# LFY1998/IPDM-PyTorch

Measured on AMD Instinct MI355X. Metric: CT slices/s (full proj+img partial-diffusion sample), higher is better.
Workload: dtype f32

## Files before the change

### ipdm-pytorch_amd/csrc/attn.hip

```cpp
#include <cstdlib>
#include "unet_kernels.h"

using namespace ipdm;

typedef float f32x16 __attribute__((ext_vector_type(16)));
typedef float f32x4 __attribute__((ext_vector_type(4)));
typedef float f32x2 __attribute__((ext_vector_type(2)));

namespace {

constexpr int KV = 64;
constexpr int KP = 68;
constexpr int VP = 68;
constexpr float LOG2E = 1.4426950408889634f;

__device__ inline int crow(int r, int h) { return (r & 3) + 8 * (r >> 2) + 4 * h; }

__device__ inline float halves_max(float x)
{
    float a = x, b = x;
    asm volatile("s_nop 1\n\tv_permlane32_swap_b32 %0, %1" : "+v"(a), "+v"(b));
    return fmaxf(a, b);
}
__device__ inline float halves_sum(float x)
{
    float a = x, b = x;
    asm volatile("s_nop 1\n\tv_permlane32_swap_b32 %0, %1" : "+v"(a), "+v"(b));
    return a + b;
}

template <int D, int QT>
__global__ void __launch_bounds__(256, 2) attention_kernel(const float *__restrict__ qkv, float *__restrict__ out,
                                                           int heads, int T, float scale)
{
    __shared__ __attribute__((aligned(16))) float k_lds[KV * KP];
    __shared__ __attribute__((aligned(16))) float v_lds[D * VP];
    const int tid = threadIdx.x, lane = tid & 63, wave = tid >> 6;
    const int l31 = lane & 31, lh = lane >> 5;
    const int bh = blockIdx.y;
    const int b = bh / heads, head = bh % heads;
    const float *qp = qkv + ((size_t)b * heads * 3 * D + (size_t)head * 3 * D) * T;
    const float *kp = qp + (size_t)D * T;
    const float *vp = qp + (size_t)2 * D * T;
    const int t0 = blockIdx.x * (128 * QT) + wave * (32 * QT);
    constexpr int HP = D / 2;

    float qreg[QT][HP];
#pragma unroll
    for (int qt = 0; qt < QT; ++qt) {
        const int t = t0 + qt * 32 + l31;
#pragma unroll
        for (int p = 0; p < HP; ++p) qreg[qt][p] = t < T ? qp[(size_t)(lh * HP + p) * T + t] * scale : 0.0f;
    }

    constexpr int CB = D / 32;
    f32x16 o[QT][CB];
#pragma unroll
    for (int qt = 0; qt < QT; ++qt)
#pragma unroll
        for (int cb = 0; cb < CB; ++cb)
#pragma unroll
            for (int r = 0; r < 16; ++r) o[qt][cb][r] = 0.0f;
    float m_run[QT], l_run[QT];
#pragma unroll
    for (int qt = 0; qt < QT; ++qt) { m_run[qt] = -INFINITY; l_run[qt] = 0.0f; }

    for (int s0 = 0; s0 < T; s0 += KV) {
        __syncthreads();
#pragma unroll
        for (int e = 0; e < (D * KV) / 256; ++e) {
            const int idx = tid + e * 256;
            const int c = idx / KV, s = idx % KV;
            const bool ok = (s0 + s) < T;
            k_lds[s * KP + c] = ok ? kp[(size_t)c * T + s0 + s] * scale : 0.0f;
            v_lds[c * VP + s] = ok ? vp[(size_t)c * T + s0 + s] : 0.0f;
        }
        __syncthreads();
#pragma unroll
        for (int sb = 0; sb < KV / 32; ++sb) {
            if (s0 + sb * 32 >= T) break;
            f32x16 sacc[QT];
#pragma unroll
            for (int qt = 0; qt < QT; ++qt)
#pragma unroll
                for (int r = 0; r < 16; ++r) sacc[qt][r] = 0.0f;
            const float *krow = k_lds + (sb * 32 + l31) * KP + lh * HP;
#pragma unroll
            for (int g = 0; g < HP / 4; ++g) {
                const f32x4 kv = *reinterpret_cast<const f32x4 *>(krow + g * 4);
#pragma unroll
                for (int j = 0; j < 4; ++j)
#pragma unroll
                    for (int qt = 0; qt < QT; ++qt)
                        sacc[qt] = __builtin_amdgcn_mfma_f32_32x32x2f32(kv[j], qreg[qt][g * 4 + j], sacc[qt], 0, 0, 0);
            }
            const bool ragged = s0 + sb * 32 + 32 > T;
#pragma unroll
            for (int qt = 0; qt < QT; ++qt) {
                if (ragged) {
#pragma unroll
                    for (int r = 0; r < 16; ++r)
                        if (s0 + sb * 32 + crow(r, lh) >= T) sacc[qt][r] = -INFINITY;
                }
                float mx = sacc[qt][0];
#pragma unroll
                for (int r = 1; r < 16; ++r) mx = fmaxf(mx, sacc[qt][r]);
                mx = halves_max(mx);
                const float m_new = fmaxf(m_run[qt], mx);
                const float mb = -m_new * LOG2E;
                const float alpha = __builtin_amdgcn_exp2f((m_run[qt] - m_new) * LOG2E);
                float rs = 0.0f;
#pragma unroll
                for (int r = 0; r < 16; ++r) {
                    sacc[qt][r] = __builtin_amdgcn_exp2f(fmaf(sacc[qt][r], LOG2E, mb));
                    rs += sacc[qt][r];
                }
                rs = halves_sum(rs);
                l_run[qt] = l_run[qt] * alpha + rs;
                m_run[qt] = m_new;
                if (__any(alpha != 1.0f)) {
#pragma unroll
                    for (int cb = 0; cb < CB; ++cb)
#pragma unroll
                        for (int r = 0; r < 16; ++r) o[qt][cb][r] *= alpha;
                }
            }
#pragma unroll
            for (int cb = 0; cb < CB; ++cb) {
                const float *vrow = v_lds + (cb * 32 + l31) * VP + sb * 32 + 4 * lh;
#pragma unroll
                for (int g = 0; g < 4; ++g) {
                    const f32x4 vv = *reinterpret_cast<const f32x4 *>(vrow + 8 * g);
#pragma unroll
                    for (int j = 0; j < 4; ++j)
#pragma unroll
                        for (int qt = 0; qt < QT; ++qt)
                            o[qt][cb] = __builtin_amdgcn_mfma_f32_32x32x2f32(vv[j], sacc[qt][4 * g + j], o[qt][cb], 0, 0, 0);
                }
            }
        }
    }
    float *op = out + ((size_t)b * heads * D + (size_t)head * D) * T;
#pragma unroll
    for (int qt = 0; qt < QT; ++qt) {
        const int t = t0 + qt * 32 + l31;
        if (t < T) {
            const float inv = 1.0f / l_run[qt];
#pragma unroll
            for (int cb = 0; cb < CB; ++cb)
#pragma unroll
                for (int r = 0; r < 16; ++r) {
                    const int c = cb * 32 + crow(r, lh);
                    op[(size_t)c * T + t] = o[qt][cb][r] * inv;
                }
        }
    }
}

struct SliceWeights { float a, b; };
__device__ inline SliceWeights slice_weights(float &M, float m_k)
{
    const float Mn = fmaxf(M, m_k);
    SliceWeights w;
    w.a = __builtin_amdgcn_exp2f((M - Mn) * LOG2E);
    w.b = __builtin_amdgcn_exp2f((m_k - Mn) * LOG2E);
    M = Mn;
    return w;
}
__device__ inline float slice_fold(float acc, float v, SliceWeights w) { return fmaf(acc, w.a, v * w.b); }

template <int D, int QT, bool ZSEQ = false>
__global__ void __launch_bounds__(512, ZSEQ ? 2 : 1) attention_ws_kernel(const float *__restrict__ qkv, float *__restrict__ out,
                                                           int heads, int T, float scale, int zsplit, float *__restrict__ part, int zseq)
{
    extern __shared__ __attribute__((aligned(16))) float smem[];
    constexpr int STAGE = KV * KP + D * VP;
    const int bh = blockIdx.y;
    const int b = bh / heads, head = bh % heads;
    const float *qp = qkv + ((size_t)b * heads * 3 * D + (size_t)head * 3 * D) * T;
    const int ntiles = (T + KV - 1) / KV;
    const int nslice = ZSEQ ? zseq : zsplit;
    const int tps = (ntiles + nslice - 1) / nslice;
    const int it0 = ZSEQ ? 0 : blockIdx.z * tps, it1 = ZSEQ ? ntiles : min(ntiles, it0 + tps);

    if (threadIdx.x >= 256) {
        const int tid = threadIdx.x - 256;
        constexpr int NE = (D * KV) / 256;
        const int s_l = tid % KV, c_l = tid / KV;
        const __amdgpu_buffer_rsrc_t rs = __builtin_amdgcn_make_buffer_rsrc((void *)qp, 0, 3 * D * T * 4, 0x00020000);
        int voff[NE];
#pragma unroll
        for (int e = 0; e < NE; ++e) voff[e] = ((c_l + (256 / KV) * e) * T + s_l) * 4;
        const int k_base = s_l * KP + c_l, v_base = c_l * VP + s_l;
        for (int it = it0; it < it1; ++it) {
            const int s0 = it * KV;
            float *k_lds = smem + (it & 1) * STAGE, *v_lds = k_lds + KV * KP;
            const bool last = s0 + KV > T;
            float kr[NE], vr[NE];
            if (!last) {
#pragma unroll
                for (int e = 0; e < NE; ++e) {
                    kr[e] = __builtin_bit_cast(float, __builtin_amdgcn_raw_buffer_load_b32(rs, voff[e], (D * T + s0) * 4, 0));
                    vr[e] = __builtin_bit_cast(float, __builtin_amdgcn_raw_buffer_load_b32(rs, voff[e], (2 * D * T + s0) * 4, 0));
                }
            } else {
#pragma unroll
                for (int e = 0; e < NE; ++e) {
                    const int vo = s0 + s_l >= T ? 0x7fffffff : voff[e];
                    kr[e] = __builtin_bit_cast(float, __builtin_amdgcn_raw_buffer_load_b32(rs, vo, (D * T + s0) * 4, 0));
                    vr[e] = __builtin_bit_cast(float, __builtin_amdgcn_raw_buffer_load_b32(rs, vo, (2 * D * T + s0) * 4, 0));
                }
            }
#pragma unroll
            for (int e = 0; e < NE; ++e) {
                k_lds[k_base + (256 / KV) * e] = kr[e];
                v_lds[v_base + (256 / KV) * e * VP] = vr[e];
            }
            __syncthreads();
        }
        return;
    }

    const int tid = threadIdx.x, lane = tid & 63, wave = tid >> 6;
    const int l31 = lane & 31, lh = lane >> 5;
    const int t0 = blockIdx.x * (128 * QT) + wave * (32 * QT);
    constexpr int HP = D / 2;
    float qreg[QT][HP];
#pragma unroll
    for (int qt = 0; qt < QT; ++qt) {
        const int t = t0 + qt * 32 + l31;
#pragma unroll
        for (int p = 0; p < HP; ++p) qreg[qt][p] = t < T ? qp[(size_t)(lh * HP + p) * T + t] * (scale * scale) : 0.0f;
    }
    constexpr int CB = D / 32;
    f32x16 o[QT][CB];
#pragma unroll
    for (int qt = 0; qt < QT; ++qt)
#pragma unroll
        for (int cb = 0; cb < CB; ++cb)
#pragma unroll
            for (int r = 0; r < 16; ++r) o[qt][cb][r] = 0.0f;
    float m_run[QT], l_run[QT];
#pragma unroll
    for (int qt = 0; qt < QT; ++qt) { m_run[qt] = -INFINITY; l_run[qt] = 0.0f; }
    static_assert(!ZSEQ || QT == 1, "attention: key slices exist for 32-query waves");
    f32x16 num[ZSEQ ? CB : 1];
    float M_all = -INFINITY, den = 0.0f;
#pragma unroll
    for (int cb = 0; cb < (ZSEQ ? CB : 1); ++cb)
#pragma unroll
        for (int r = 0; r < 16; ++r) num[cb][r] = 0.0f;
    int slice_end = it0 + tps;

    for (int it = it0; it < it1; ++it) {
        const int s0 = it * KV;
        __syncthreads();
        const float *k_lds = smem + (it & 1) * STAGE, *v_lds = k_lds + KV * KP;
#pragma unroll
        for (int sb = 0; sb < KV / 32; ++sb) {
            if (s0 + sb * 32 >= T) break;
            f32x16 sacc[QT];
#pragma unroll
            for (int qt = 0; qt < QT; ++qt)
#pragma unroll
                for (int r = 0; r < 16; ++r) sacc[qt][r] = 0.0f;
            const float *krow = k_lds + (sb * 32 + l31) * KP + lh * HP;
#pragma unroll
            for (int g = 0; g < HP / 4; ++g) {
                const f32x4 kv = *reinterpret_cast<const f32x4 *>(krow + g * 4);
#pragma unroll
                for (int j = 0; j < 4; ++j)
#pragma unroll
                    for (int qt = 0; qt < QT; ++qt)
                        sacc[qt] = __builtin_amdgcn_mfma_f32_32x32x2f32(kv[j], qreg[qt][g * 4 + j], sacc[qt], 0, 0, 0);
            }
            const bool ragged = s0 + sb * 32 + 32 > T;
#pragma unroll
            for (int qt = 0; qt < QT; ++qt) {
                if (ragged) {
#pragma unroll
                    for (int r = 0; r < 16; ++r)
                        if (s0 + sb * 32 + crow(r, lh) >= T) sacc[qt][r] = -INFINITY;
                }
                float mx = sacc[qt][0];
#pragma unroll
                for (int r = 1; r < 16; ++r) mx = fmaxf(mx, sacc[qt][r]);
                mx = halves_max(mx);
                const float m_new = fmaxf(m_run[qt], mx);
                const float mb = -m_new * LOG2E;
                const float alpha = __builtin_amdgcn_exp2f((m_run[qt] - m_new) * LOG2E);
                f32x2 rs2 = {0.0f, 0.0f};
#pragma unroll
                for (int r = 0; r < 16; r += 2) {
                    f32x2 v = f32x2{sacc[qt][r], sacc[qt][r + 1]} * LOG2E + mb;
                    v[0] = __builtin_amdgcn_exp2f(v[0]);
                    v[1] = __builtin_amdgcn_exp2f(v[1]);
                    sacc[qt][r] = v[0];
                    sacc[qt][r + 1] = v[1];
                    rs2 += v;
                }
                float rs = halves_sum(rs2[0] + rs2[1]);
                l_run[qt] = l_run[qt] * alpha + rs;
                m_run[qt] = m_new;
                if (__any(alpha != 1.0f)) {
#pragma unroll
                    for (int cb = 0; cb < CB; ++cb)
#pragma unroll
                        for (int r = 0; r < 16; ++r) o[qt][cb][r] *= alpha;
                }
            }
#pragma unroll
            for (int cb = 0; cb < CB; ++cb) {
                const float *vrow = v_lds + (cb * 32 + l31) * VP + sb * 32 + 4 * lh;
#pragma unroll
                for (int g = 0; g < 4; ++g) {
                    const f32x4 vv = *reinterpret_cast<const f32x4 *>(vrow + 8 * g);
#pragma unroll
                    for (int j = 0; j < 4; ++j)
#pragma unroll
                        for (int qt = 0; qt < QT; ++qt)
                            o[qt][cb] = __builtin_amdgcn_mfma_f32_32x32x2f32(vv[j], sacc[qt][4 * g + j], o[qt][cb], 0, 0, 0);
                }
            }
        }
        if constexpr (ZSEQ) if (it + 1 == slice_end || it + 1 == it1) {
            const SliceWeights w = slice_weights(M_all, m_run[0]);
            den = slice_fold(den, l_run[0], w);
#pragma unroll
            for (int cb = 0; cb < CB; ++cb)
#pragma unroll
                for (int r = 0; r < 16; ++r) { num[cb][r] = slice_fold(num[cb][r], o[0][cb][r], w); o[0][cb][r] = 0.0f; }
            m_run[0] = -INFINITY;
            l_run[0] = 0.0f;
            slice_end += tps;
        }
    }
    if (zsplit > 1) {
        float *pp = part + ((size_t)blockIdx.z * gridDim.y + bh) * (D + 2) * T;
#pragma unroll
        for (int qt = 0; qt < QT; ++qt) {
            const int t = t0 + qt * 32 + l31;
            if (t < T) {
#pragma unroll
                for (int cb = 0; cb < CB; ++cb)
#pragma unroll
                    for (int r = 0; r < 16; ++r) pp[(size_t)(cb * 32 + crow(r, lh)) * T + t] = o[qt][cb][r];
                if (lh == 0) { pp[(size_t)D * T + t] = m_run[qt]; pp[(size_t)(D + 1) * T + t] = l_run[qt]; }
            }
        }
        return;
    }
    float *op = out + ((size_t)b * heads * D + (size_t)head * D) * T;
#pragma unroll
    for (int qt = 0; qt < QT; ++qt) {
        const int t = t0 + qt * 32 + l31;
        if (t < T) {
            constexpr bool seq = ZSEQ;
            const float inv = 1.0f / (seq ? den : l_run[qt]);
#pragma unroll
            for (int cb = 0; cb < CB; ++cb)
#pragma unroll
                for (int r = 0; r < 16; ++r) {
                    const int c = cb * 32 + crow(r, lh);
                    op[(size_t)c * T + t] = (seq ? num[seq ? cb : 0][r] : o[qt][cb][r]) * inv;
                }
        }
    }
}

template <int D>
__global__ void __launch_bounds__(256) attention_combine_kernel(const float *__restrict__ part, float *__restrict__ out, int T, int Z, int ntiles)
{
    const int t = blockIdx.x * 256 + threadIdx.x, bh = blockIdx.y, c0 = blockIdx.z * 16;
    if (t >= T) return;
    const size_t slice = (size_t)gridDim.y * (D + 2) * T;
    const float *p = part + (size_t)bh * (D + 2) * T;
    const int tps = (ntiles + Z - 1) / Z;
    SliceWeights w[8];
    float M = -INFINITY, den = 0.0f;
#pragma unroll
    for (int z = 0; z < 8; ++z)
        if (z < Z && z * tps < ntiles) {
            w[z] = slice_weights(M, p[z * slice + (size_t)D * T + t]);
            den = slice_fold(den, p[z * slice + (size_t)(D + 1) * T + t], w[z]);
        }
    const float inv = 1.0f / den;
#pragma unroll 4
    for (int c = c0; c < c0 + 16; ++c) {
        float acc = 0.0f;
#pragma unroll
        for (int z = 0; z < 8; ++z)
            if (z < Z && z * tps < ntiles) acc = slice_fold(acc, p[z * slice + (size_t)c * T + t], w[z]);
        out[((size_t)bh * D + c) * T + t] = acc * inv;
    }
}

int attention_kv_split(int B, int heads, int d, int T)
{
    const bool off = opt(OPT_ATTN_NO_KVSPLIT) != 0;
    (void)B;
    if (off || d != 64) return 1;
    const long wg = (long)cdiv(T, 128) * heads;
    if (wg > 128) return 1;
    const int ntiles = cdiv(T, KV);
    int Z = wg <= 32 ? 8 : (wg <= 64 ? 4 : 2);
    if (Z > ntiles / 2) Z = ntiles / 2;
    return Z < 2 ? 1 : Z;
}

}

namespace ipdm {

size_t attention_scratch_floats(int B, int heads, int d, int T)
{
    const int Z = attention_kv_split(B, heads, d, T);
    return Z > 1 ? (size_t)Z * B * heads * (d + 2) * T : 0;
}

int attention_launch(const float *qkv, float *out, int B, int heads, int d, int T, hipStream_t st, float *scratch)
{
    IPDM_REQUIRE(qkv && out && B > 0 && heads > 0 && T > 0, "attention: bad argument");
    if (d != 64 && d != 32) { set_error("attention: head dim %d unsupported (kernel is specialised for 64 and 32)", d); return IPDM_ERR_UNSUPPORTED; }
    const float scale = (float)(1.0 / sqrt(sqrt((double)d)));
    const bool prof = prof_enabled();
    if (prof) prof_before(2, st);
    const bool legacy = opt(OPT_ATTN_LEGACY) != 0;
    if (d == 64 && !legacy) {
        constexpr size_t lds = (size_t)2 * (KV * KP + 64 * VP) * sizeof(float);
        if (int rc = ensure_dynamic_lds((const void *)attention_ws_kernel<64, 1>, lds)) return rc;
        if (int rc = ensure_dynamic_lds((const void *)attention_ws_kernel<64, 2>, lds)) return rc;
        if (int rc = ensure_dynamic_lds((const void *)attention_ws_kernel<64, 1, true>, lds)) return rc;
        const long wg2 = (long)cdiv(T, 256) * B * heads, wg1 = (long)cdiv(T, 128) * B * heads;
        const auto eff = [](long wg) { return (double)wg / (double)(((wg + 255) / 256) * 256); };
        const int Z = scratch ? attention_kv_split(B, heads, d, T) : 1;
        const bool q2 = Z == 1 && wg2 >= 256 && eff(wg2) >= eff(wg1) - 0.03;
        const bool no_seq = opt(OPT_ATTN_NO_ZSEQ) != 0;
        const bool seq = Z >= 4 && !no_seq && wg1 >= 192;
        dim3 grid(cdiv(T, q2 ? 256 : 128), B * heads, seq ? 1 : Z);
        if (q2) hipLaunchKernelGGL((attention_ws_kernel<64, 2>), grid, dim3(512), lds, st, qkv, out, heads, T, scale, 1, (float *)nullptr, 1);
        else if (seq) hipLaunchKernelGGL((attention_ws_kernel<64, 1, true>), grid, dim3(512), lds, st, qkv, out, heads, T, scale, 1, (float *)nullptr, Z);
        else hipLaunchKernelGGL((attention_ws_kernel<64, 1>), grid, dim3(512), lds, st, qkv, out, heads, T, scale, Z, scratch, 1);
        if (Z > 1 && !seq)
            hipLaunchKernelGGL((attention_combine_kernel<64>), dim3(cdiv(T, 256), B * heads, 4), dim3(256), 0, st, scratch, out, T, Z, cdiv(T, KV));
    } else if (d == 64) {
        const long wg2 = (long)cdiv(T, 256) * B * heads;
        const bool q2 = wg2 >= 512 && (wg2 % 512 == 0 || wg2 >= 4 * 512);
        dim3 grid(cdiv(T, q2 ? 256 : 128), B * heads);
        if (q2) hipLaunchKernelGGL((attention_kernel<64, 2>), grid, dim3(256), 0, st, qkv, out, heads, T, scale);
        else hipLaunchKernelGGL((attention_kernel<64, 1>), grid, dim3(256), 0, st, qkv, out, heads, T, scale);
    } else {
        dim3 grid(cdiv(T, 128), B * heads);
        hipLaunchKernelGGL((attention_kernel<32, 1>), grid, dim3(256), 0, st, qkv, out, heads, T, scale);
    }
    if (prof) prof_after(2, 4.0 * B * heads * (double)T * T * d, st);
    IPDM_LAUNCH_CHECK();
    return IPDM_OK;
}

}

extern "C" int32_t ipdm_attention_kernel_code(int32_t d)
{
    return (d == 64 && !ipdm::opt(ipdm::OPT_ATTN_LEGACY)) ? 1 : 0;
}

extern "C" int ipdm_op_attention(const float *d_qkv, float *d_out, int32_t B, int32_t heads, int32_t d, int32_t T,
                                 void *stream)
{
    float *scratch = nullptr;
    if (ipdm::attention_scratch_floats(B, heads, d, T)) {
        IPDM_HIP_CHECK(hipMalloc((void **)&scratch, ipdm::attention_scratch_floats(B, heads, d, T) * sizeof(float)));
    }
    const int rc = ipdm::attention_launch(d_qkv, d_out, B, heads, d, T, (hipStream_t)stream, scratch);
    if (scratch) {
        (void)hipStreamSynchronize((hipStream_t)stream);
        (void)hipFree(scratch);
    }
    return rc;
}
```

### ipdm-pytorch_amd/csrc/common.h

```cpp
#pragma once
#include <hip/hip_runtime.h>
#include <cstdarg>
#include <cstdio>
#include <cstring>
#include <string>
#include <vector>
#include "../../include/ipdm_hip.h"

namespace ipdm {

void set_error(const char *fmt, ...);

#define IPDM_HIP_CHECK(expr)                                                                   \
    do {                                                                                       \
        hipError_t e_ = (expr);                                                                \
        if (e_ != hipSuccess) {                                                                \
            ipdm::set_error("%s failed: %s (%s:%d)", #expr, hipGetErrorString(e_), __FILE__,  \
                            __LINE__);                                                         \
            return IPDM_ERR_HIP;                                                               \
        }                                                                                      \
    } while (0)

#define IPDM_REQUIRE(cond, ...)                   \
    do {                                          \
        if (!(cond)) {                            \
            ipdm::set_error(__VA_ARGS__);         \
            return IPDM_ERR_INVALID;              \
        }                                         \
    } while (0)

#define IPDM_LAUNCH_CHECK() IPDM_HIP_CHECK(hipGetLastError())

static inline int cdiv(long a, long b) { return (int)((a + b - 1) / b); }
static inline size_t align_up(size_t v, size_t a) { return (v + a - 1) / a * a; }

enum Opt {
    OPT_CONV_NO_UP2,
    OPT_CONV_NO_WUP2,
    OPT_CONV_LEGACY, OPT_CONV1X1_LEGACY, OPT_CONVS2_LEGACY,
    OPT_CONV_NO_DIRECT, OPT_DIRECT_NO_PLANAR, OPT_DIRECT_MAX_CIN, OPT_DIRECT_NO_S2, OPT_DIRECT_NO_SKIP_FUSE,
    OPT_CONV_DBG, OPT_CONV_VEC4_STRICT, OPT_CONV_NO_SPLITK, OPT_CONV_NO_WINO, OPT_WINO_V1, OPT_WINO2_MIN_TILES, OPT_CONV1X1_NO_QUARTER, OPT_CONV_NO_PW, OPT_PW_ITEM, OPT_PW_FORCE,
    OPT_CONV_NM,
    OPT_GN_TWO_STAGE, OPT_GN_UNFUSED,
    OPT_UNET_TRANSPOSE,
    OPT_ATTN_NO_KVSPLIT, OPT_ATTN_LEGACY, OPT_ATTN_NO_ZSEQ,
    OPT_ART_PER_VIEW,
    OPT_CONV_BF16X3,
    OPT_COUNT
};
int opt(Opt o);
bool opt_per_call(int o);
const char *opt_name(int o);
void opt_snapshot(int (&dst)[OPT_COUNT]);
int opt_changed_since(const int (&rec)[OPT_COUNT]);
std::vector<int> opt_per_call_values();

int ensure_dynamic_lds(const void *kernel, size_t bytes);
int device_cu_count();

__device__ inline double wave_sum(double v)
{
#pragma unroll
    for (int o = 32; o > 0; o >>= 1) v += __shfl_down(v, o, 64);
    return v;
}
__device__ inline float wave_sum(float v)
{
#pragma unroll
    for (int o = 32; o > 0; o >>= 1) v += __shfl_down(v, o, 64);
    return v;
}
__device__ inline float wave_max(float v)
{
#pragma unroll
    for (int o = 32; o > 0; o >>= 1) v = fmaxf(v, __shfl_down(v, o, 64));
    return v;
}

}
```

### ipdm-pytorch_amd/csrc/common.hip

```cpp
#include <cctype>
#include <cstdlib>
#include <mutex>
#include <strings.h>
#include <set>
#include <utility>
#include "common.h"

namespace ipdm {
static thread_local char g_err[512] = "";
void set_error(const char *fmt, ...)
{
    va_list ap;
    va_start(ap, fmt);
    vsnprintf(g_err, sizeof(g_err), fmt, ap);
    va_end(ap);
}

namespace {
std::mutex g_attr_mu;
std::set<std::pair<const void *, int>> g_attr_done;
int g_cus[64];
}

namespace {
struct OptDef { const char *name; int def; bool per_call; int lo = 0, hi = 1; };
const OptDef g_opt_def[OPT_COUNT] = {
    {"conv_no_up2", 0, true},
    {"conv_no_wup2", 0, true},
    {"conv_legacy", 0, false}, {"conv1x1_legacy", 0, false}, {"convs2_legacy", 0, false},
    {"conv_no_direct", 0, false}, {"direct_no_planar", 0, false},
    {"direct_max_cin", 160, false, 0, 160},
    {"direct_no_s2", 0, false}, {"direct_no_skip_fuse", 0, true},
    {"conv_dbg", 0, true, 0, 0x3ff}, {"conv_vec4_strict", 0, false}, {"conv_no_splitk", 0, false},
    {"conv_no_wino", 0, true}, {"wino_v1", 0, true}, {"wino2_min_tiles", 192, true, 0, 1 << 24},
    {"conv1x1_no_quarter", 0, true}, {"conv_no_pw", 0, true}, {"pw_item", 0, true, 0, 2}, {"pw_force", 0, true}, {"conv_nm", 0, true, 0, 2},
    {"gn_two_stage", 0, true}, {"gn_unfused", 0, true},
    {"unet_transpose", -1, true, -1, 1},
    {"attn_no_kvsplit", 0, false}, {"attn_legacy", 0, false}, {"attn_no_zseq", 0, true},
    {"art_per_view", 0, true},
    {"conv_bf16x3", 0, true},
};
bool opt_value_ok(int i, int v)
{
    return v >= g_opt_def[i].lo && v <= g_opt_def[i].hi;
}
std::mutex g_opt_mu;
int g_opt_val[OPT_COUNT];
bool g_opt_init = false;

void opt_init_locked()
{
    if (g_opt_init) return;
    for (int i = 0; i < OPT_COUNT; ++i) {
        char env[64] = "IPDM_";
        size_t n = 5;
        for (const char *c = g_opt_def[i].name; *c && n + 1 < sizeof(env); ++c) env[n++] = (char)toupper((unsigned char)*c);
        env[n] = 0;
        const char *e = getenv(env);
        g_opt_val[i] = g_opt_def[i].def;
        if (e) {
            char *end = nullptr;
            const long v = strtol(e, &end, 10);
            const int want = (end != e) ? (int)v : 1;
            if (opt_value_ok(i, want)) g_opt_val[i] = want;
            else fprintf(stderr, "libipdm_hip: %s=%s is outside the option's range [%d, %d]: ignored\n", env, e, g_opt_def[i].lo, g_opt_def[i].hi);
        }
    }
    g_opt_init = true;
}
}

int opt(Opt o)
{
    std::lock_guard<std::mutex> lk(g_opt_mu);
    opt_init_locked();
    return g_opt_val[o];
}
bool opt_per_call(int o) { return g_opt_def[o].per_call; }
const char *opt_name(int o) { return g_opt_def[o].name; }
void opt_snapshot(int (&dst)[OPT_COUNT])
{
    std::lock_guard<std::mutex> lk(g_opt_mu);
    opt_init_locked();
    for (int i = 0; i < OPT_COUNT; ++i) dst[i] = g_opt_val[i];
}
std::vector<int> opt_per_call_values()
{
    std::lock_guard<std::mutex> lk(g_opt_mu);
    opt_init_locked();
    std::vector<int> v;
    for (int i = 0; i < OPT_COUNT; ++i)
        if (g_opt_def[i].per_call) v.push_back(g_opt_val[i]);
    return v;
}
int opt_changed_since(const int (&rec)[OPT_COUNT])
{
    std::lock_guard<std::mutex> lk(g_opt_mu);
    opt_init_locked();
    for (int i = 0; i < OPT_COUNT; ++i)
        if (!g_opt_def[i].per_call && g_opt_val[i] != rec[i]) return i;
    return -1;
}
static int opt_find(const char *name)
{
    if (!name) return -1;
    if (!strncmp(name, "IPDM_", 5) || !strncmp(name, "ipdm_", 5)) name += 5;
    for (int i = 0; i < OPT_COUNT; ++i)
        if (!strcasecmp(name, g_opt_def[i].name)) return i;
    return -1;
}

int ensure_dynamic_lds(const void *kernel, size_t bytes)
{
    int dev = 0;
    IPDM_HIP_CHECK(hipGetDevice(&dev));
    std::lock_guard<std::mutex> lk(g_attr_mu);
    if (g_attr_done.count({kernel, dev})) return IPDM_OK;
    IPDM_HIP_CHECK(hipFuncSetAttribute(kernel, hipFuncAttributeMaxDynamicSharedMemorySize, (int)bytes));
    g_attr_done.insert({kernel, dev});
    return IPDM_OK;
}

int device_cu_count()
{
    int dev = 0, v = 0;
    if (hipGetDevice(&dev) != hipSuccess || dev < 0 || dev >= 64) return 256;
    std::lock_guard<std::mutex> lk(g_attr_mu);
    if (!g_cus[dev])
        g_cus[dev] = (hipDeviceGetAttribute(&v, hipDeviceAttributeMultiprocessorCount, dev) == hipSuccess && v > 0) ? v : 256;
    return g_cus[dev];
}
}

extern "C" const char *ipdm_last_error(void) { return ipdm::g_err; }
extern "C" int ipdm_abi_version(void) { return IPDM_ABI_VERSION; }

extern "C" int ipdm_set_option(const char *name, int value)
{
    const int i = ipdm::opt_find(name);
    IPDM_REQUIRE(i >= 0, "ipdm_set_option: unknown option '%s'", name ? name : "(null)");
    IPDM_REQUIRE(ipdm::opt_value_ok(i, value), "ipdm_set_option: %s = %d is outside [%d, %d]", ipdm::g_opt_def[i].name, value,
                 ipdm::g_opt_def[i].lo, ipdm::g_opt_def[i].hi);
    std::lock_guard<std::mutex> lk(ipdm::g_opt_mu);
    ipdm::opt_init_locked();
    ipdm::g_opt_val[i] = value;
    return IPDM_OK;
}

extern "C" int ipdm_get_option(const char *name, int *value)
{
    const int i = ipdm::opt_find(name);
    IPDM_REQUIRE(i >= 0 && value, "ipdm_get_option: unknown option '%s'", name ? name : "(null)");
    *value = ipdm::opt((ipdm::Opt)i);
    return IPDM_OK;
}
```

### ipdm-pytorch_amd/csrc/unet_kernels.h

```cpp
#pragma once
#include <vector>
#include "common.h"

namespace ipdm {

struct GnTileSrc { const float *stats = nullptr; int rows = 0, C = 0; };
struct GnTileArgs {
    GnTileSrc src[2];
    int nsrc = 1, B = 0;
    long HW = 0;
    int groups = 0;
    const float *gamma = nullptr, *beta = nullptr;
    float eps = 1e-5f;
    double *partials = nullptr;
    float *scale = nullptr, *shift = nullptr;
};

struct ConvArgs {
    const float *x1, *x2;
    int C1, C2, B;
    int Hs, Ws;
    int H, W;
    int upsample;
    float scale_y, scale_x;
    const float *w;
    int cout_pad;
    int w_interleave = 0;
    const float *bias;
    int Cout, ksize, stride;
    int Ho, Wo;
    int act;
    const float *gn_scale, *gn_shift;
    const float *res;
    float *out;
    int tiles_x, tiles_y, co_tiles;
    float *stats = nullptr;
    int stats_rows = 0;
    float *split_ws = nullptr;
    int ksplit = 1;
    const float *w_up2 = nullptr;
    const float *w_wup2 = nullptr;
    const float *w_wino = nullptr;
    const float *sk_x1 = nullptr, *sk_x2 = nullptr, *sk_w = nullptr;
    int sk_C1 = 0, sk_C2 = 0, sk_cout_pad = 0, sk_planar = 0;
    int x1_planar = 0;
    int up2 = 0;
    int dbg = 0;
    unsigned long long *dbg_buf = nullptr;
};

int conv2d_launch(const ConvArgs &a, hipStream_t st);
int conv_kernel_code(const ConvArgs &a);
int conv2d_ws_launch(const ConvArgs &a, hipStream_t st);
bool conv_direct_eligible(const ConvArgs &a);
int conv2d_direct_launch(const ConvArgs &a, hipStream_t st);
bool conv_nm_eligible(const ConvArgs &a);
int conv2d_nm_launch(const ConvArgs &a, hipStream_t st);
int conv_k_chunk();
int conv_ws_k_chunk(int ks, int interleave);

constexpr int PROF_CLASSES = 8;
bool prof_enabled();
void prof_before(int cls, hipStream_t st);
void prof_after(int cls, double flops, hipStream_t st);
int conv_weight_interleave(int Cout, int ks, int stride);
void conv_pack_weights(const float *w, int Cout, int Cin, int ks, int interleave, std::vector<float> &packed, int &cin_pad, int &cout_pad);

struct GnArgs {
    const float *x1, *x2;
    int C1, C2, B;
    long HW;
    int groups;
    const float *gamma, *beta;
    float eps;
    double *partials;
    float *scale, *shift;
    int split = 0;
};
constexpr int GN_SPLIT = 64;
int gn_tiles_launch(const GnTileArgs &a, hipStream_t st);
int conv_stats_rows(const ConvArgs &a);
int conv_split(const ConvArgs &a);
size_t conv_split_ws_bytes(const ConvArgs &a);
constexpr int SPLIT_PIX = 2048;
int conv_ws_stats_rows(const ConvArgs &a);
bool conv_up2_eligible(const ConvArgs &a);
bool conv_wino_eligible(const ConvArgs &a);
bool conv_wup2_shape_ok(int Cout, int Cin);
bool conv_wup2_eligible(const ConvArgs &a);
int conv2d_wup2_launch(const ConvArgs &orig, hipStream_t st, int prof_cls);
void conv_pack_weights_wup2(const float *w, int Cout, int Cin, std::vector<float> &packed);
bool conv_wino_shape_ok(int Cout, int Cin, int ks, int stride, int interleave);
int conv2d_wino_launch(const ConvArgs &a, hipStream_t st);
int conv_wino_split(const ConvArgs &a);
bool conv_wino2_eligible(const ConvArgs &a);
int conv2d_wino2_launch(const ConvArgs &prepared, hipStream_t st);
bool conv_wino3_eligible(const ConvArgs &prepared);
int conv2d_wino3_launch(const ConvArgs &prepared, hipStream_t st);
void conv_pack_weights_wino(const float *w, int Cout, int Cin, std::vector<float> &packed);
bool conv_ws_planar_ok(const ConvArgs &a);
bool conv_direct_skip_ok(const ConvArgs &a);
bool conv_direct_up2_eligible(const ConvArgs &a);
bool conv_planar_ok(const ConvArgs &a);
void conv_pack_weights_up2(const float *w, int Cout, int Cin, int interleave, std::vector<float> &packed);
int planar_to_linear_launch(const float *src, float *dst, long planes, int H, int W, hipStream_t st);
int conv_ws_split(const ConvArgs &a);
bool conv_pw_eligible(const ConvArgs &a);
bool conv_pw_layer_ok(const ConvArgs &a);
bool conv_pw_stats_layer(const ConvArgs &a);
int conv_pw_stats_rows(const ConvArgs &a);
int conv2d_pw_launch(const ConvArgs &a, hipStream_t st);
int conv_direct_stats_rows(const ConvArgs &a);
size_t gn_partials_bytes(int B, int groups);
int gn_stats_launch(const GnArgs &a, hipStream_t st);

int attention_launch(const float *qkv, float *out, int B, int heads, int d, int T, hipStream_t st, float *scratch = nullptr);
size_t attention_scratch_floats(int B, int heads, int d, int T);

int temb_launch(const float *freqs, int mc, int t, const float *w0, const float *b0, const float *w2, const float *b2,
                float *tmp, float *silu_emb, hipStream_t st);
int gemv_bias_launch(const float *W, const float *b, const float *base, const float *v, float *y, int rows, int K,
                     hipStream_t st);

}
```

Measured before the change: 2.042.

## Add bf16x3 split-precision MFMA attention kernel as default d=64 path

Adds a new attention kernel that splits fp32 Q, K, V and P into three bf16 parts and emulates fp32 matmuls with six bf16 MFMA products per tile. The fp32 MFMA path it replaces has lower matrix throughput. Producer waves convert K and V into the split bf16 layout in shared memory, with a 32-key tile and double buffering. The old exact fp32 kernel stays behind a new opt-out flag; the new path costs extra conversion work and some accuracy versus true fp32.

```diff
diff --git a/ipdm-pytorch_amd/csrc/attn.hip b/ipdm-pytorch_amd/csrc/attn.hip
--- a/ipdm-pytorch_amd/csrc/attn.hip
+++ b/ipdm-pytorch_amd/csrc/attn.hip
@@ -1,7 +1,9 @@
 #include <cstdlib>
 #include "unet_kernels.h"
+#include "attn_common.h"
 
 using namespace ipdm;
+using namespace ipdm::attn;
 
 typedef float f32x16 __attribute__((ext_vector_type(16)));
 typedef float f32x4 __attribute__((ext_vector_type(4)));
@@ -12,22 +14,6 @@
 constexpr int KV = 64;
 constexpr int KP = 68;
 constexpr int VP = 68;
-constexpr float LOG2E = 1.4426950408889634f;
-
-__device__ inline int crow(int r, int h) { return (r & 3) + 8 * (r >> 2) + 4 * h; }
-
-__device__ inline float halves_max(float x)
-{
-    float a = x, b = x;
-    asm volatile("s_nop 1\n\tv_permlane32_swap_b32 %0, %1" : "+v"(a), "+v"(b));
-    return fmaxf(a, b);
-}
-__device__ inline float halves_sum(float x)
-{
-    float a = x, b = x;
-    asm volatile("s_nop 1\n\tv_permlane32_swap_b32 %0, %1" : "+v"(a), "+v"(b));
-    return a + b;
-}
 
 template <int D, int QT>
 __global__ void __launch_bounds__(256, 2) attention_kernel(const float *__restrict__ qkv, float *__restrict__ out,
@@ -157,17 +143,6 @@
     }
 }
 
-struct SliceWeights { float a, b; };
-__device__ inline SliceWeights slice_weights(float &M, float m_k)
-{
-    const float Mn = fmaxf(M, m_k);
-    SliceWeights w;
-    w.a = __builtin_amdgcn_exp2f((M - Mn) * LOG2E);
-    w.b = __builtin_amdgcn_exp2f((m_k - Mn) * LOG2E);
-    M = Mn;
-    return w;
-}
-__device__ inline float slice_fold(float acc, float v, SliceWeights w) { return fmaf(acc, w.a, v * w.b); }
 
 template <int D, int QT, bool ZSEQ = false>
 __global__ void __launch_bounds__(512, ZSEQ ? 2 : 1) attention_ws_kernel(const float *__restrict__ qkv, float *__restrict__ out,
@@ -426,7 +401,15 @@
     const bool prof = prof_enabled();
     if (prof) prof_before(2, st);
     const bool legacy = opt(OPT_ATTN_LEGACY) != 0;
-    if (d == 64 && !legacy) {
+    const bool exact = opt(OPT_ATTN_EXACT_F32) != 0;
+    if (d == 64 && !legacy && !exact) {
+        const int Z = scratch ? attention_kv_split(B, heads, d, T) : 1;
+        const long wg1 = (long)cdiv(T, 128) * B * heads;
+        const bool seq = Z >= 4 && opt(OPT_ATTN_NO_ZSEQ) == 0 && wg1 >= 192;
+        attention_bx3_launch(qkv, out, B, heads, T, scale, Z, seq, scratch, st);
+        if (Z > 1 && !seq)
+            hipLaunchKernelGGL((attention_combine_kernel<64>), dim3(cdiv(T, 256), B * heads, 4), dim3(256), 0, st, scratch, out, T, Z, cdiv(T, KV));
+    } else if (d == 64 && !legacy) {
         constexpr size_t lds = (size_t)2 * (KV * KP + 64 * VP) * sizeof(float);
         if (int rc = ensure_dynamic_lds((const void *)attention_ws_kernel<64, 1>, lds)) return rc;
         if (int rc = ensure_dynamic_lds((const void *)attention_ws_kernel<64, 2>, lds)) return rc;
@@ -462,7 +445,8 @@
 
 extern "C" int32_t ipdm_attention_kernel_code(int32_t d)
 {
-    return (d == 64 && !ipdm::opt(ipdm::OPT_ATTN_LEGACY)) ? 1 : 0;
+    if (d != 64 || ipdm::opt(ipdm::OPT_ATTN_LEGACY)) return 0;
+    return ipdm::opt(ipdm::OPT_ATTN_EXACT_F32) ? 1 : 2;
 }
 
 extern "C" int ipdm_op_attention(const float *d_qkv, float *d_out, int32_t B, int32_t heads, int32_t d, int32_t T,
diff --git a/ipdm-pytorch_amd/csrc/attn_bx3.hip b/ipdm-pytorch_amd/csrc/attn_bx3.hip
--- /dev/null
+++ b/ipdm-pytorch_amd/csrc/attn_bx3.hip
@@ -0,0 +1,280 @@
+#include "unet_kernels.h"
+#include "attn_common.h"
+
+using namespace ipdm;
+using namespace ipdm::attn;
+
+typedef float f32x16 __attribute__((ext_vector_type(16)));
+typedef unsigned u32x4 __attribute__((ext_vector_type(4)));
+typedef __bf16 bf16x8 __attribute__((ext_vector_type(8)));
+typedef __bf16 bf16x2 __attribute__((ext_vector_type(2)));
+
+namespace {
+
+constexpr int D = 64;
+constexpr int KT = 32;
+constexpr int KP = 72;
+constexpr int VP = 40;
+constexpr int KPLANE = KT * KP, VPLANE = D * VP;
+constexpr int STAGE = 3 * KPLANE + 3 * VPLANE;
+
+__device__ inline unsigned pk_bf16(float a, float b)
+{
+    return __builtin_bit_cast(unsigned, bf16x2{(__bf16)a, (__bf16)b});
+}
+struct Split3 { unsigned h[3]; };
+__device__ inline Split3 split3(float a, float b)
+{
+    Split3 s;
+    s.h[0] = pk_bf16(a, b);
+    const float ra = a - __builtin_bit_cast(float, s.h[0] << 16), rb = b - __builtin_bit_cast(float, s.h[0] & 0xffff0000u);
+    s.h[1] = pk_bf16(ra, rb);
+    const float qa = ra - __builtin_bit_cast(float, s.h[1] << 16), qb = rb - __builtin_bit_cast(float, s.h[1] & 0xffff0000u);
+    s.h[2] = pk_bf16(qa, qb);
+    return s;
+}
+
+__device__ inline f32x16 mma(u32x4 a, u32x4 b, f32x16 c)
+{
+    return __builtin_amdgcn_mfma_f32_32x32x16_bf16(__builtin_bit_cast(bf16x8, a), __builtin_bit_cast(bf16x8, b), c, 0, 0, 0);
+}
+template <bool FIRST>
+__device__ inline f32x16 mma6(const u32x4 (&a)[3], const u32x4 (&b)[3], f32x16 c)
+{
+    if (FIRST) {
+        const f32x16 zero = {0, 0, 0, 0, 0, 0, 0, 0, 0, 0, 0, 0, 0, 0, 0, 0};
+        c = mma(a[0], b[2], zero);
+        asm volatile("" ::"v"(a[0]), "v"(b[2]));
+    } else {
+        c = mma(a[0], b[2], c);
+    }
+    c = mma(a[2], b[0], c);
+    c = mma(a[1], b[1], c);
+    c = mma(a[0], b[1], c);
+    c = mma(a[1], b[0], c);
+    return mma(a[0], b[0], c);
+}
+
+template <bool ZSEQ>
+__global__ void __launch_bounds__(384, 3) attention_bx3_kernel(const float *__restrict__ qkv, float *__restrict__ out, int heads, int T,
+                                                                float scale, int zsplit, float *__restrict__ part, int zseq)
+{
+    __shared__ __attribute__((aligned(16))) unsigned short lds[2 * STAGE];
+    const int bh = blockIdx.y;
+    const int b = bh / heads, head = bh % heads;
+    const float *qp = qkv + ((size_t)b * heads * 3 * D + (size_t)head * 3 * D) * T;
+    const int ntiles = (T + KT - 1) / KT;
+    const int nslice = ZSEQ ? zseq : zsplit;
+    const int tps = 2 * (((T + 63) / 64 + nslice - 1) / nslice);
+    const int it0 = ZSEQ ? 0 : blockIdx.z * tps, it1 = ZSEQ ? ntiles : min(ntiles, it0 + tps);
+
+    if (__builtin_amdgcn_readfirstlane(threadIdx.x >> 6) >= 4) {
+        const int tid = threadIdx.x - 256;
+        const __amdgpu_buffer_rsrc_t rs = __builtin_amdgcn_make_buffer_rsrc((void *)qp, 0, 3 * D * T * 4, 0x00020000);
+        int ks[2], kg[2], koff[2], vg[2], vc[2], vkey[2], voff[2];
+#pragma unroll
+        for (int n = 0; n < 2; ++n) {
+            const int idx = tid + 128 * n;
+            ks[n] = idx & 31;
+            kg[n] = idx >> 5;
+            koff[n] = (8 * kg[n] * T + ks[n]) * 4;
+            vg[n] = idx & 3;
+            vc[n] = idx >> 2;
+            vkey[n] = 16 * (vg[n] >> 1) + 4 * (vg[n] & 1);
+            voff[n] = (vc[n] * T + vkey[n]) * 4;
+        }
+        float kr[2][8], vr[2][8];
+        const auto load = [&](int it) {
+            const int s0 = it * KT;
+            if (s0 + KT <= T) {
+#pragma unroll
+                for (int n = 0; n < 2; ++n)
+#pragma unroll
+                    for (int e = 0; e < 8; ++e) {
+                        kr[n][e] = __builtin_bit_cast(float, __builtin_amdgcn_raw_buffer_load_b32(rs, koff[n], (D * T + s0 + e * T) * 4, 0));
+                        vr[n][e] = __builtin_bit_cast(float, __builtin_amdgcn_raw_buffer_load_b32(rs, voff[n], (2 * D * T + s0 + 8 * (e >> 2) + (e & 3)) * 4, 0));
+                    }
+            } else {
+#pragma unroll
+                for (int n = 0; n < 2; ++n)
+#pragma unroll
+                    for (int e = 0; e < 8; ++e) {
+                        const int ko = s0 + ks[n] >= T ? 0x7fffffff : koff[n];
+                        const int vo = s0 + vkey[n] + 8 * (e >> 2) + (e & 3) >= T ? 0x7fffffff : voff[n];
+                        kr[n][e] = __builtin_bit_cast(float, __builtin_amdgcn_raw_buffer_load_b32(rs, ko, (D * T + s0 + e * T) * 4, 0));
+                        vr[n][e] = __builtin_bit_cast(float, __builtin_amdgcn_raw_buffer_load_b32(rs, vo, (2 * D * T + s0 + 8 * (e >> 2) + (e & 3)) * 4, 0));
+                    }
+            }
+        };
+        const auto store = [&](int it) {
+            unsigned short *st = lds + (it & 1) * STAGE;
+#pragma unroll
+            for (int n = 0; n < 2; ++n) {
+                u32x4 hk[3], hv[3];
+#pragma unroll
+                for (int e = 0; e < 8; e += 2) {
+                    const Split3 sk = split3(kr[n][e], kr[n][e + 1]), sv = split3(vr[n][e], vr[n][e + 1]);
+#pragma unroll
+                    for (int p = 0; p < 3; ++p) { hk[p][e / 2] = sk.h[p]; hv[p][e / 2] = sv.h[p]; }
+                }
+#pragma unroll
+                for (int p = 0; p < 3; ++p) {
+                    *reinterpret_cast<u32x4 *>(st + p * KPLANE + ks[n] * KP + 8 * kg[n]) = hk[p];
+                    *reinterpret_cast<u32x4 *>(st + 3 * KPLANE + p * VPLANE + vc[n] * VP + 8 * vg[n]) = hv[p];
+                }
+            }
+        };
+        if (it0 < it1) load(it0);
+        for (int it = it0; it < it1; ++it) {
+            store(it);
+            if (it + 1 < it1) load(it + 1);
+            __syncthreads();
+        }
+        return;
+    }
+
+    const int tid = threadIdx.x, lane = tid & 63, wave = tid >> 6;
+    const int l31 = lane & 31, lh = lane >> 5;
+    const int t = blockIdx.x * 128 + wave * 32 + l31;
+    u32x4 q[4][3];
+#pragma unroll
+    for (int kb = 0; kb < 4; ++kb) {
+        float x[8];
+#pragma unroll
+        for (int e = 0; e < 8; ++e) x[e] = t < T ? qp[(size_t)(16 * kb + 8 * lh + e) * T + t] * (scale * scale) : 0.0f;
+#pragma unroll
+        for (int e = 0; e < 8; e += 2) {
+            const Split3 s = split3(x[e], x[e + 1]);
+#pragma unroll
+            for (int p = 0; p < 3; ++p) q[kb][p][e / 2] = s.h[p];
+        }
+    }
+    f32x16 o[2];
+#pragma unroll
+    for (int cb = 0; cb < 2; ++cb)
+#pragma unroll
+        for (int r = 0; r < 16; ++r) o[cb][r] = 0.0f;
+    float m_run = -INFINITY, l_run = 0.0f;
+    f32x16 num[ZSEQ ? 2 : 1];
+    float M_all = -INFINITY, den = 0.0f;
+#pragma unroll
+    for (int cb = 0; cb < (ZSEQ ? 2 : 1); ++cb)
+#pragma unroll
+        for (int r = 0; r < 16; ++r) num[cb][r] = 0.0f;
+    int slice_end = it0 + tps;
+    u32x4 v[2][3] = {}, pp[2][3] = {};
+    const auto reserve = [&]() {
+        asm volatile("" ::"v"(v[0][0]), "v"(v[0][1]), "v"(v[0][2]), "v"(v[1][0]), "v"(v[1][1]), "v"(v[1][2]), "v"(pp[1][0]), "v"(pp[1][1]), "v"(pp[1][2]));
+    };
+
+    for (int it = it0; it < it1; ++it) {
+        const int s0 = it * KT;
+        __syncthreads();
+        reserve();
+        const unsigned short *st = lds + (it & 1) * STAGE;
+        f32x16 sacc;
+        u32x4 k[3];
+        {
+            const unsigned short *krow = st + l31 * KP + 8 * lh;
+#pragma unroll
+            for (int kb = 0; kb < 4; ++kb) {
+#pragma unroll
+                for (int p = 0; p < 3; ++p) k[p] = *reinterpret_cast<const u32x4 *>(krow + p * KPLANE + 16 * kb);
+                sacc = kb == 0 ? mma6<true>(k, q[kb], sacc) : mma6<false>(k, q[kb], sacc);
+            }
+        }
+        __builtin_amdgcn_sched_barrier(0);
+        if (s0 + KT > T) {
+#pragma unroll
+            for (int r = 0; r < 16; ++r)
+                if (s0 + crow(r, lh) >= T) sacc[r] = -INFINITY;
+        }
+        float mx = sacc[0];
+#pragma unroll
+        for (int r = 1; r < 16; ++r) mx = fmaxf(mx, sacc[r]);
+        mx = halves_max(mx);
+        const float m_new = fmaxf(m_run, mx);
+        const float alpha = __builtin_amdgcn_exp2f((m_run - m_new) * LOG2E);
+        float rs0 = 0.0f, rs1 = 0.0f;
+#pragma unroll
+        for (int r = 0; r < 16; r += 2) {
+            sacc[r] = __builtin_amdgcn_exp2f((sacc[r] - m_new) * LOG2E);
+            sacc[r + 1] = __builtin_amdgcn_exp2f((sacc[r + 1] - m_new) * LOG2E);
+            rs0 += sacc[r];
+            rs1 += sacc[r + 1];
+        }
+        const float rs = halves_sum(rs0 + rs1);
+        asm volatile("" ::"v"(k[0]), "v"(k[1]), "v"(k[2]));
+        l_run = l_run * alpha + rs;
+        m_run = m_new;
+        if (__any(alpha != 1.0f)) {
+#pragma unroll
+            for (int cb = 0; cb < 2; ++cb)
+#pragma unroll
+                for (int r = 0; r < 16; ++r) o[cb][r] *= alpha;
+        }
+#pragma unroll
+        for (int kb = 0; kb < 2; ++kb)
+#pragma unroll
+            for (int e = 0; e < 8; e += 2) {
+                const Split3 s = split3(sacc[8 * kb + e], sacc[8 * kb + e + 1]);
+#pragma unroll
+                for (int p = 0; p < 3; ++p) pp[kb][p][e / 2] = s.h[p];
+            }
+        __builtin_amdgcn_sched_barrier(0);
+#pragma unroll
+        for (int cb = 0; cb < 2; ++cb) {
+            const unsigned short *vrow = st + 3 * KPLANE + (cb * 32 + l31) * VP + 8 * lh;
+#pragma unroll
+            for (int kb = 0; kb < 2; ++kb)
+#pragma unroll
+                for (int p = 0; p < 3; ++p) v[kb][p] = *reinterpret_cast<const u32x4 *>(vrow + p * VPLANE + 16 * kb);
+#pragma unroll
+            for (int kb = 0; kb < 2; ++kb) o[cb] = mma6<false>(v[kb], pp[kb], o[cb]);
+        }
+        __builtin_amdgcn_sched_barrier(0);
+        if constexpr (ZSEQ) if (it + 1 == slice_end || it + 1 == it1) {
+            const SliceWeights w = slice_weights(M_all, m_run);
+            den = slice_fold(den, l_run, w);
+#pragma unroll
+            for (int cb = 0; cb < 2; ++cb)
+#pragma unroll
+                for (int r = 0; r < 16; ++r) { num[cb][r] = slice_fold(num[cb][r], o[cb][r], w); o[cb][r] = 0.0f; }
+            m_run = -INFINITY;
+            l_run = 0.0f;
+            slice_end += tps;
+        }
+    }
+    if (t >= T) { reserve(); return; }
+    if (zsplit > 1) {
+        float *pq = part + ((size_t)blockIdx.z * gridDim.y + bh) * (D + 2) * T;
+#pragma unroll
+        for (int cb = 0; cb < 2; ++cb)
+#pragma unroll
+            for (int r = 0; r < 16; ++r) pq[(size_t)(cb * 32 + crow(r, lh)) * T + t] = o[cb][r];
+        if (lh == 0) { pq[(size_t)D * T + t] = m_run; pq[(size_t)(D + 1) * T + t] = l_run; }
+        reserve();
+        return;
+    }
+    float *op = out + ((size_t)b * heads * D + (size_t)head * D) * T;
+    const float inv = 1.0f / (ZSEQ ? den : l_run);
+#pragma unroll
+    for (int cb = 0; cb < 2; ++cb)
+#pragma unroll
+        for (int r = 0; r < 16; ++r) op[(size_t)(cb * 32 + crow(r, lh)) * T + t] = (ZSEQ ? num[ZSEQ ? cb : 0][r] : o[cb][r]) * inv;
+    reserve();
+}
+
+}
+
+namespace ipdm {
+
+void attention_bx3_launch(const float *qkv, float *out, int B, int heads, int T, float scale, int Z, bool seq, float *scratch,
+                          hipStream_t st)
+{
+    const dim3 grid(cdiv(T, 128), B * heads, seq ? 1 : Z);
+    if (seq) hipLaunchKernelGGL((attention_bx3_kernel<true>), grid, dim3(384), 0, st, qkv, out, heads, T, scale, 1, (float *)nullptr, Z);
+    else hipLaunchKernelGGL((attention_bx3_kernel<false>), grid, dim3(384), 0, st, qkv, out, heads, T, scale, Z, scratch, 1);
+}
+
+}
diff --git a/ipdm-pytorch_amd/csrc/attn_common.h b/ipdm-pytorch_amd/csrc/attn_common.h
--- /dev/null
+++ b/ipdm-pytorch_amd/csrc/attn_common.h
@@ -0,0 +1,37 @@
+#pragma once
+#include <hip/hip_runtime.h>
+
+namespace ipdm {
+namespace attn {
+
+constexpr float LOG2E = 1.4426950408889634f;
+
+__device__ inline int crow(int r, int h) { return (r & 3) + 8 * (r >> 2) + 4 * h; }
+
+__device__ inline float halves_max(float x)
+{
+    float a = x, b = x;
+    asm volatile("s_nop 1\n\tv_permlane32_swap_b32 %0, %1" : "+v"(a), "+v"(b));
+    return fmaxf(a, b);
+}
+__device__ inline float halves_sum(float x)
+{
+    float a = x, b = x;
+    asm volatile("s_nop 1\n\tv_permlane32_swap_b32 %0, %1" : "+v"(a), "+v"(b));
+    return a + b;
+}
+
+struct SliceWeights { float a, b; };
+__device__ inline SliceWeights slice_weights(float &M, float m_k)
+{
+    const float Mn = fmaxf(M, m_k);
+    SliceWeights w;
+    w.a = __builtin_amdgcn_exp2f((M - Mn) * LOG2E);
+    w.b = __builtin_amdgcn_exp2f((m_k - Mn) * LOG2E);
+    M = Mn;
+    return w;
+}
+__device__ inline float slice_fold(float acc, float v, SliceWeights w) { return fmaf(acc, w.a, v * w.b); }
+
+}
+}
diff --git a/ipdm-pytorch_amd/csrc/common.h b/ipdm-pytorch_amd/csrc/common.h
--- a/ipdm-pytorch_amd/csrc/common.h
+++ b/ipdm-pytorch_amd/csrc/common.h
@@ -46,6 +46,7 @@
     OPT_ATTN_NO_KVSPLIT, OPT_ATTN_LEGACY, OPT_ATTN_NO_ZSEQ,
     OPT_ART_PER_VIEW,
     OPT_CONV_BF16X3,
+    OPT_ATTN_EXACT_F32,
     OPT_COUNT
 };
 int opt(Opt o);
diff --git a/ipdm-pytorch_amd/csrc/common.hip b/ipdm-pytorch_amd/csrc/common.hip
--- a/ipdm-pytorch_amd/csrc/common.hip
+++ b/ipdm-pytorch_amd/csrc/common.hip
@@ -39,6 +39,7 @@
     {"attn_no_kvsplit", 0, false}, {"attn_legacy", 0, false}, {"attn_no_zseq", 0, true},
     {"art_per_view", 0, true},
     {"conv_bf16x3", 0, true},
+    {"attn_exact_f32", 0, true},
 };
 bool opt_value_ok(int i, int v)
 {
diff --git a/ipdm-pytorch_amd/csrc/unet_kernels.h b/ipdm-pytorch_amd/csrc/unet_kernels.h
--- a/ipdm-pytorch_amd/csrc/unet_kernels.h
+++ b/ipdm-pytorch_amd/csrc/unet_kernels.h
@@ -116,6 +116,8 @@
 
 int attention_launch(const float *qkv, float *out, int B, int heads, int d, int T, hipStream_t st, float *scratch = nullptr);
 size_t attention_scratch_floats(int B, int heads, int d, int T);
+void attention_bx3_launch(const float *qkv, float *out, int B, int heads, int T, float scale, int Z, bool seq, float *scratch,
+                          hipStream_t st);
 
 int temb_launch(const float *freqs, int mc, int t, const float *w0, const float *b0, const float *w2, const float *b2,
                 float *tmp, float *silu_emb, hipStream_t st);
```

Result: faster. 2.094, median of 6 (+2.5%).
